# vrettasm/VGPA

Hardware: AMD Instinct MI355X
Metric: fwd+bwd sweeps/sec (free-energy+grad eval), Lorenz96 D=40 N=1000 (higher is better)
Workload: dtype f64; 1 GPU; Lorenz96 D=40, RK4, Np=1001 (BASELINE configs[2]); batch_per_gpu=512, kernels=mfma

## Files before the change

vgpa_amd/csrc/ode_sym_impl.h:

```cpp
#pragma once
#include <type_traits>
#include <utility>
#include "ode_mfma_impl.h"

namespace vgpa {
namespace sym {

using mfma::cdiv;
using mfma::cmax;
using mfma::cmin;
using mfma::d2_t;
using mfma::ldg;
using mfma::ldu;
using mfma::n_stages;
using mfma::settle;
using mfma::stage_op;
using mfma::stg;
using mfma::OP_M;
using mfma::OP_R;
using mfma::OP_X;

constexpr int kMaxNB = 16;

struct Run { int c, j0, j1; };
// ... 21 lines not shown
        if (j == v || (cov & pair_bit(v, j))) continue;
        if (a < 0) a = j;
        else if (b < 0) b = j;
      }
      if (b < 0) break;
      cov |= pair_bit(v, a) | pair_bit(v, b);
      if (n == want) res = Run{v, a, b};
      n++;
    }
  }
  for (int v = 0; v < nsb; v++)
    for (int j = v + 1; j < nsb; j++) {
      if (cov & pair_bit(v, j)) continue;
      cov |= pair_bit(v, j);
      if (n == want) res = Run{v, j, -1};
      n++;
    }
  if (count) *count = n;
  return res;
}

__host__ __device__ constexpr int sym_run_count(int nsb) {
  int n = 0;
  (void)sym_run(nsb, -2, &n);
  return n;
}

constexpr int kCoverPat[4][2] = {{0, 2}, {0, 3}, {1, 2}, {1, 3}};
constexpr int kCoverMaps[4][4][4] = {
    {{1, 8, 6, 1}, {2, 6, 7, 3}, {6, 5, 5, 4}, {9, 2, 5, 2}},
    {{9, 9, 8, 0}, {8, 1, 1, 2}, {8, 1, 1, 2}, {4, 5, 0, 5}},
    {{6, 9, 3, 6}, {4, 0, 5, 9}, {4, 0, 5, 9}, {0, 7, 4, 3}},
    {{8, 1, 7, 8}, {6, 7, 2, 3}, {6, 7, 2, 3}, {7, 3, 4, 0}}};
constexpr int kCoverUsed[4] = {0xB, 0xF, 0xF, 0xF};
constexpr bool kCoverAlias[4] = {false, true, true, true};
constexpr int kCoverLoopSlot = 2;
__host__ __device__ constexpr bool cover_slot_used(int w, int s) { return (kCoverUsed[w] >> s) & 1; }
__host__ __device__ constexpr bool cover_owner(int w, int s, int q) {
  const int I = kCoverMaps[w][kCoverPat[s][0]][q], J = kCoverMaps[w][kCoverPat[s][1]][q];
  const int lo = I < J ? I : J, hi = I < J ? J : I;
  for (int w2 = 0; w2 <= w; w2++)
    for (int s2 = 0; s2 < 4; s2++)
      for (int q2 = 0; q2 < 4; q2++) {
        if (!cover_slot_used(w2, s2)) continue;
        if (w2 == w && (s2 > s || (s2 == s && q2 >= q))) return true;
        const int I2 = kCoverMaps[w2][kCoverPat[s2][0]][q2], J2 = kCoverMaps[w2][kCoverPat[s2][1]][q2];
        if ((I2 < J2 ? I2 : J2) == lo && (I2 < J2 ? J2 : I2) == hi) return false;
      }
  return true;
}
struct CoverOwnerTab { unsigned char m[4][4]; };
__host__ __device__ constexpr CoverOwnerTab cover_owner_tab() {
  CoverOwnerTab t{};
  for (int w = 0; w < 4; w++)
    for (int s = 0; s < 4; s++) {
      unsigned char bits = 0;
      for (int q = 0; q < 4; q++)
        if (cover_slot_used(w, s) && cover_owner(w, s, q)) bits = (unsigned char)(bits | (1u << q));
      t.m[w][s] = bits;
    }
  return t;
}
__device__ constexpr CoverOwnerTab kCoverOwner = cover_owner_tab();
__host__ __device__ constexpr int cover_pairs_owned() {
  int n = 0;
  for (int w = 0; w < 4; w++)
    for (int s = 0; s < 4; s++)
      for (int q = 0; q < 4; q++) n += (cover_slot_used(w, s) && cover_owner(w, s, q)) ? 1 : 0;
  return n;
}
static_assert(cover_pairs_owned() == 55, "the fragment cover must own every block pair of the 10 x 10 upper triangle exactly once");
__host__ __device__ constexpr bool cover_diagonals_in_loop_units() {
  for (int w = 0; w < 4; w++)
    for (int s = 0; s < 4; s++)
      for (int q = 0; q < 4; q++) {
        if (!cover_slot_used(w, s)) continue;
        const bool diag = kCoverMaps[w][kCoverPat[s][0]][q] == kCoverMaps[w][kCoverPat[s][1]][q];
        const bool loop = kCoverAlias[w] && s == kCoverLoopSlot;
        if (diag != loop) return false;
      }
  return !cover_slot_used(0, kCoverLoopSlot);
}
static_assert(cover_diagonals_in_loop_units(), "single-chain loop units: every diagonal block in slot 2 of a triangle wave, slot 2 of the rectangle wave unused");

template <int NB_>
struct SGeo {
  static constexpr int NB = NB_;
  static constexpr int NW = 4, NT = 64 * NW;
  static constexpr int P = 4 * NB;
  static constexpr int NSB = (NB + 1) / 2;
  static constexpr int KKE = 2 * NSB;
  static constexpr int PP = 4 * KKE;
  static constexpr int RP = 2 * KKE;
  static constexpr int NKP = NSB;
  static constexpr int LD = 32 * cdiv(2 * PP - 16, 32) + 16;
  static constexpr int XS = RP * LD;
  static constexpr int NRUNS = sym_run_count(NSB);
  static constexpr int NR = cdiv(NRUNS, 4);
  static constexpr int MAXS = 2 * NR;
  static constexpr int XV = PP + 4;
  static constexpr int NPARTF = cmin(NT / PP, RP);
  static constexpr int RPP = cdiv(RP, NPARTF);
  static constexpr int NPF = cmin(NPARTF, cdiv(RP, RPP));
  static constexpr int NCB = PP / 4;
  static constexpr int NPARTB = cmin(NT / RP, NCB);
  static constexpr int CBP = cdiv(NCB, NPARTB);
  static constexpr int NPART = cmax(NPF, NPARTB);
  static constexpr int PV = NPART * PP;
  static constexpr int NIT = cdiv((P / 2) * P, NT);
  static constexpr int NTILE = cdiv(P / 2, 8) * cdiv(P, 8);
  static constexpr int NITF = cdiv(NTILE, NW);
  static constexpr size_t LDS_DOUBLES = (size_t)4 * XS + NW * XV + 2 * PV + 2 * NT;
  static_assert(NPARTF >= 1 && NPARTB >= 1, "dimension too large for the workgroup");
};

template <int NB>
__host__ __device__ constexpr int elem_off(int k, int c) {
  return (k >> 1) * SGeo<NB>::LD + 2 * (c ^ ((k >> 1) & 3)) + (k & 1);
}
template <int NB>
__host__ __device__ constexpr int unit_off(int p, int c) {
  return p * SGeo<NB>::LD + 2 * (c ^ (p & 3));
}

template <int NB>
struct ItemTab {
  static constexpr int NIT = SGeo<NB>::NIT;
  int lo[NIT];
  unsigned g0[NIT];
  unsigned g1[NIT];
  bool two[NIT];
  bool st0[NIT], st1[NIT];
};
template <int NB>
__device__ __forceinline__ void build_items(int D, int tid, ItemTab<NB>& T, bool packed_lower = false) {
  using g = SGeo<NB>;
#pragma unroll
  for (int q = 0; q < g::NIT; q++) {
    const int e = tid + g::NT * q;
    const int p = e / g::P, c = e - p * g::P;
    const bool ok = 2 * p < D && c < D;
    T.lo[q] = ok ? unit_off<NB>(p, c) : -1;
    T.g0[q] = ok ? 8u * (unsigned)(2 * p * D + c) : 0u;
    T.two[q] = ok && 2 * p + 1 < D;
    T.g1[q] = T.two[q] ? T.g0[q] + 8u * (unsigned)D : T.g0[q];
    T.st0[q] = ok; T.st1[q] = T.two[q];
    if (packed_lower) {
      const int r0 = 2 * p, r1 = 2 * p + 1;
      T.st0[q] = ok && c <= r0;
      T.st1[q] = T.two[q] && c <= r1;
      T.g0[q] = T.st0[q] ? 8u * (unsigned)(r0 * (r0 + 1) / 2 + c) : 0u;
      T.g1[q] = T.st1[q] ? 8u * (unsigned)(r1 * (r1 + 1) / 2 + c) : 0u;
    }
  }
}

template <int NB>
struct TileTab {
  static constexpr int NIT = SGeo<NB>::NITF;
  int lo[NIT];
  unsigned g0[NIT], g1[NIT];
  bool two[NIT];
};
template <int NB>
__device__ __forceinline__ void build_tiles(int D, int wave, int lane, TileTab<NB>& T) {
  using g = SGeo<NB>;
// ... 263 lines not shown
      for (int u = 0; u < 6; u++) wr1(eo_o[u], __builtin_fma(m2dt, gacc[u], -(uu[u / 3] * mm[u % 3])));
    } else {
#pragma unroll
      for (int u = 0; u < 7; u++) wr1(eo_o[u], __builtin_fma(m2dt, gacc[u], -(uu[u < 3 ? u : 2] * mm[u < 3 ? 0 : u - 2])));
    }
  };
  auto out = [&](int tg) {
    double* gA = gbase + (size_t)tg * DD;
    double v[NOUT];
#pragma unroll
    for (int q = 0; q < NOUT; q++) v[q] = rd1(ol[q]);
#pragma unroll
    for (int q = 0; q < NOUT; q++) stgo(gA, oo[q], v[q]);
  };
  using I0 = std::integral_constant<int, 0>; using I1 = std::integral_constant<int, 1>; using I2 = std::integral_constant<int, 2>;
  using I4 = std::integral_constant<int, 4>; using I5 = std::integral_constant<int, 5>;

  constexpr int kPrio = 3;
  auto step = [&](int k, auto set_, auto hp_, auto hp2_) {
    constexpr int SET = decltype(set_)::value;
    constexpr bool HP = decltype(hp_)::value, HP2 = decltype(hp2_)::value;
    using CUR = std::integral_constant<int, SET>; using PRV = std::integral_constant<int, SET ^ 1>;
    opaque_tables();
    if (HP) settle_loads();
    if (HP2) out(tidx(k - 2));
    __builtin_amdgcn_sched_barrier(0);
    build(CUR{});
    __builtin_amdgcn_sched_barrier(0);
    if (HP) prod(PRV{}, I0{}, I1{});
    lds_barrier();
    band_u(CUR{}, tidx(k));
    prefetch(tidx(k + 1));
    __builtin_amdgcn_sched_barrier(0);
    if (HP) prod(PRV{}, I1{}, I2{});
    lds_barrier();
    if (HP) prod(PRV{}, I2{}, I4{});
    lds_barrier();
    if (HP) { prod(PRV{}, I4{}, I5{}); __builtin_amdgcn_sched_barrier(0); epilogue(PRV{}); }
    lds_barrier();
  };
  auto drain = [&](auto set_) {
    constexpr int SET = decltype(set_)::value;
    using CUR = std::integral_constant<int, SET>; using PRV = std::integral_constant<int, SET ^ 1>;
    if (n_steps > 0) settle_loads();
    if (n_steps > 1) out(tidx(n_steps - 2));
    build(CUR{});
    if (n_steps > 0) prod(PRV{}, I0{}, I5{});
    lds_barrier();
    if (n_steps > 0) epilogue(PRV{});
    band_u(CUR{}, tidx(n_steps));
    lds_barrier();
    if (n_steps > 0) out(tidx(n_steps - 1));
    prod(CUR{}, I0{}, I5{});
    lds_barrier();
    epilogue(CUR{});
    lds_barrier();
    out(tidx(n_steps));
  };

  __builtin_amdgcn_s_setprio(kPrio);
  __syncthreads();
  prefetch(tidx(0));
  settle_loads();
  __syncthreads();
  using F = std::false_type; using T = std::true_type;
  int k = 0;
  if (n_steps > 0) { step(0, I0{}, F{}, F{}); k = 1; }
  if (n_steps > 1) { step(1, I1{}, T{}, F{}); k = 2; }
  for (; k + 1 < n_steps; k += 2) { step(k, I0{}, T{}, T{}); step(k + 1, I1{}, T{}, T{}); }
  if (k < n_steps) step(k, I0{}, T{}, T{});
  if (n_steps & 1) drain(I1{});
  else drain(I0{});
}

template <int METHOD, bool FWD, int NB, bool DENSEJ, int GR, int WPE, bool QOUT = false, bool HLP = false, bool GF = false, bool H2 = false, bool PJ = false>
__global__ void __attribute__((amdgpu_flat_work_group_size(256 * ((GF || H2) ? 3 : (HLP ? 2 : 1)), 256 * ((GF || H2) ? 3 : (HLP ? 2 : 1))), amdgpu_waves_per_eu(WPE, WPE))) k_ode_sym(OdeArgs a) {
#pragma clang fp contract(fast)
  extern __shared__ __attribute__((aligned(16))) double smem[];
  using g = SGeo<NB>;
  constexpr int NT = g::NT;
  constexpr int NS = n_stages<METHOD>(), NR = g::NR, MAXS = g::MAXS, LD = g::LD, NKP = g::NKP;
  constexpr bool COVER = (GR == 0);
  static_assert(!COVER || (g::NSB == 5 && g::MAXS == 4), "the fragment cover is built for 33 <= D <= 40");
  static_assert(!HLP || COVER, "helper waves: fragment-cover kernels");
  static_assert(!GF || (HLP && QOUT && !FWD && !DENSEJ && METHOD == VGPA_ODE_RK4), "fused gradient assembly: backward RK4 helper-wave kernels with Q'' on");
  static_assert(!H2 || (HLP && !GF), "two helper roles: helper-wave kernels without the gradient waves");
  static_assert(!PJ || (!FWD && !DENSEJ), "per-problem constant matrix jump: backward kernels with sparse jumps");
  constexpr int NITS = FWD ? g::NITF : g::NIT;
  constexpr int JSEC = NS > 1 ? 1 : 0;
  constexpr int LSTG = (NS == 4 && HLP) ? 3 : JSEC;
  constexpr double sixth = 1.0 / 6.0;
  const int role = HLP ? (int)threadIdx.x / NT : 0;
  const bool helper = role >= 1;
  const int tid = (int)threadIdx.x - role * NT, lane = tid & 63, wave = tid >> 6;
  const int wq = wave & 3;
  const int prob = (int)blockIdx.x;
  const int D = a.D, Np = a.Np, DD = a.D * a.D, n_steps = a.Np - 1;
  const double dt = a.dt, h = 0.5 * a.dt;
  const double q_scale = a.q_scale_v ? lds_const(a.q_scale_v, prob) : a.q_scale;
  double* const Xb0 = smem;
  double* const Xb1 = Xb0 + g::XS;
  double* const Rb = Xb1 + g::XS;
  double* const Mb = Rb + g::XS;
  double* const xvw = Mb + g::XS + wave * g::XV;
  double* const pvb = Mb + g::XS + g::NW * g::XV;
  double* const trash = pvb + 2 * g::PV + 2 * tid;
  using gl = GradLds<NB>;
  constexpr int GLDS = GF ? gl::DOUBLES : 0;
  if constexpr (GF) {
    if (role == 2) { grad_waves<NB>(a, smem, (int)threadIdx.x - 2 * NT); return; }
  }
  double* const gLam = smem + g::LDS_DOUBLES + gl::LAM;
  for (int i = tid; i < (int)g::LDS_DOUBLES + GLDS; i += NT) smem[i] = 0.0;
  static_assert(!QOUT || (!FWD && (METHOD == VGPA_ODE_RK2 || METHOD == VGPA_ODE_RK4)), "Q'' is stored by the backward mid-point kernels");
  auto tidx =[&](int i) { return FWD ? i : Np - 1 - i; };
  auto tclamp = [&](int i) { return tidx(i <= n_steps ? i : n_steps); };

  const int r4 = lane >> 4, bq = (lane >> 2) & 3, c4 = lane & 3, bi = bq >> 1, bj = bq & 1;
  int colI[NR], colJ[MAXS], offD[MAXS], offM[MAXS];
  int colm[4] = {0, 0, 0, 0};
  unsigned gofs[MAXS];
  bool own[MAXS], wd[MAXS], wm[MAXS];
  const int cov_used = COVER ? kCoverUsed[wq] : 0;
  const bool loop_diag = r4 == c4;
  const int loop_src = 16 * c4 + 4 * bq + r4;
  if constexpr (COVER) {
#pragma unroll
    for (int m = 0; m < 4; m++) colm[m] = 2 * ((4 * kCoverMaps[wq][m][bq] + c4) ^ r4);
#pragma unroll
    for (int s = 0; s < MAXS; s++) {
      const int Ib = kCoverMaps[wq][kCoverPat[s][0]][bq], Jb = kCoverMaps[wq][kCoverPat[s][1]][bq];
      const int row = 4 * Ib + r4, col = 4 * Jb + c4;
      const bool first = (kCoverOwner.m[wq][s] >> bq) & 1u;
      const bool act = ((cov_used >> s) & 1) && first && (Ib != Jb || row <= col);
      offD[s] = elem_off<NB>(row, col);
      offM[s] = elem_off<NB>(col, row);
      wd[s] = act;
      wm[s] = act && row != col;
      own[s] = act && row < D && col < D;
      gofs[s] = own[s] ? 8u * (unsigned)(row <= col ? row * D + col : col * D + row) : 0u;
      if (!FWD && a.ds_packed) gofs[s] = own[s] ? 8u * (unsigned)(row <= col ? tri_off(col) + row : tri_off(row) + col) : 0u;
      colJ[s] = 0;
    }
#pragma unroll
    for (int rl = 0; rl < NR; rl++) colI[rl] = 0;
  } else {
#pragma unroll
  for (int rl = 0; rl < NR; rl++) {
    const Run run = sym_run(g::NSB, wave + 4 * rl, nullptr);
    const bool rv = run.c >= 0;
    const int c = rv ? run.c : 0;
    const int Ib = 2 * c + bi;
    colI[rl] = 2 * ((4 * Ib + c4) ^ r4);
#pragma unroll
    for (int t = 0; t < 2; t++) {
      const int s = 2 * rl + t;
      const int jr = t ? run.j1 : run.j0;
      const bool valid = rv && jr >= 0;
      const int j = valid ? jr : 0;
      const int Jb = 2 * j + bj;
      const int row = 4 * Ib + r4, col = 4 * Jb + c4;
      colJ[s] = 2 * ((4 * Jb + c4) ^ r4);
      offD[s] = elem_off<NB>(row, col);
      offM[s] = elem_off<NB>(col, row);
      const bool act = valid && (c != j || row <= col);
      wd[s] = act;
      wm[s] = act && row != col;
      own[s] = act && row < D && col < D;
      gofs[s] = own[s] ? 8u * (unsigned)(row <= col ? row * D + col : col * D + row) : 0u;
      if (!FWD && a.ds_packed) gofs[s] = own[s] ? 8u * (unsigned)(row <= col ? tri_off(col) + row : tri_off(row) + col) : 0u;
    }
  }
  }
  const bool spk = FWD && a.s_packed;
  const int MS = spk ? D * (D + 1) / 2 : DD;
  ItemTab<NB> IT;
  build_items<NB>(D, tid, IT, spk);
  TileTab<NB> TT;
  if (FWD) build_tiles<NB>(D, wave, lane, TT);

  const double* A = a.A + (size_t)prob * a.strideA;
  d2_t an[NITS];
  auto load_a = [&](const double* At) {
#pragma unroll
    for (int q = 0; q < NITS; q++) {
      an[q][0] = ldgo(At, FWD ? TT.g0[q] : IT.g0[q]);
      an[q][1] = ldgo(At, FWD ? TT.g1[q] : IT.g1[q]);
    }
  };
  auto unit_ptr = [&](double* buf, int q) -> d2_t* {
    const int lo = FWD ? TT.lo[q] : IT.lo[q];
    return reinterpret_cast<d2_t*>(lo >= 0 ? buf + lo : trash);
  };
  auto mask_a = [&]() {
#pragma unroll
    for (int q = 0; q < NITS; q++)
      if (!(FWD ? TT.two[q] : IT.two[q])) an[q][1] = 0.0;
  };
  auto store_a = [&](double* buf, const d2_t (&v)[NITS]) {
#pragma unroll
    for (int q = 0; q < NITS; q++) *unit_ptr(buf, q) = v[q];
  };
  const int GS = (!FWD && a.ds_packed) ? D * (D + 1) / 2 : DD;
  const double* G = FWD ? a.Sigma + (size_t)prob * a.Sigma_stride : a.dEs + (size_t)prob * Np * GS;
  double* const mout = (FWD ? a.S : a.psi) + (size_t)prob * Np * (spk ? D * (D + 1) / 2 : DD);
  double xk[MAXS], acc[MAXS], fc[MAXS], fn[MAXS], fnn[MAXS];
#pragma unroll
  for (int s = 0; s < MAXS; s++) {
// ... 4 lines not shown
    acc[s] = 0.0;
  }

  const bool vl = lane < D;
  unsigned lane8 = vl ? 8u * (unsigned)lane : 0u;
  double* const xv_mine = vl ? xvw + lane : trash;
  const double* cin = FWD ? a.b + (size_t)prob * a.strideB : a.dEm + (size_t)prob * Np * D;
  double* const vout = (FWD ? a.m : a.lam) + (size_t)prob * Np * D;
  auto vec = [&](int t) { return (size_t)t * D; };
  const bool sparse_j = !FWD && !DENSEJ && a.obs_idx && a.jm_sparse;
  const int32_t* const obs_idx = a.obs_idx + (size_t)prob * a.obs_idx_stride;
  auto jump_vector = [&](int t, int n_obs) -> double {
    if (!FWD && DENSEJ) return ldg(a.jm_dense + ((size_t)prob * Np + t) * D, lane8);
    if (sparse_j && __builtin_amdgcn_readfirstlane(n_obs) >= 0) return ldg(a.jm_sparse + ((size_t)prob * a.n_obs + n_obs) * D, lane8);
    return 0.0;
  };
  double vk = FWD ? ldg(a.m0 + (size_t)prob * a.m0_stride, lane8) : 0.0, v1 = 0.0;
  double c0 = ldg(cin + vec(tidx(0)), lane8), c1 = ldg(cin + vec(tclamp(1)), lane8), c2 = 0.0;
  int n_obs_cur = sparse_j ? ldu(obs_idx, tclamp(1)) : -1, n_obs_next = sparse_j ? ldu(obs_idx, tclamp(2)) : -1, n_obs_nn = -1;
  double jm = n_steps >= 1 ? jump_vector(tidx(1), n_obs_cur) : 0.0, jm_next = 0.0;

  __syncthreads();
#pragma unroll
  for (int s = 0; s < MAXS; s++) {
    if (FWD) {
      *(wd[s] ? Xb0 + offD[s] : trash) = xk[s];
      *(wm[s] ? Xb0 + offM[s] : trash) = xk[s];
    }
  }
  *xv_mine = vk;
  load_a(A + (size_t)tidx(0) * DD);
  mask_a();
  store_a(Rb, an);
  load_a(A + (size_t)tclamp(1) * DD);
#pragma unroll
  for (int s = 0; s < MAXS; s++) { settle(fc[s]); settle(fn[s]); settle(xk[s]); }
  settle(c0); settle(c1); settle(vk); settle(jm);
#pragma unroll
  for (int q = 0; q < NITS; q++) settle(an[q]);
  mask_a();
  auto mask_f = [&](int s, double v) -> double {
    if (COVER && s == kCoverLoopSlot) v *= loop_diag ? 0.5 : 1.0;
    return own[s] ? -v : 0.0;
  };
#pragma unroll
  for (int s = 0; s < MAXS; s++) { fc[s] = mask_f(s, fc[s]); if (!FWD) fn[s] = mask_f(s, fn[s]); }
  __syncthreads();

  auto store_vector = [&](int t) {
    if (wave == 0 && vl) stgo(vout + vec(t), lane8, vk);
  };
  auto store_items = [&](const d2_t (&v)[g::NIT], int t, bool with_vector = true) {
    double* so = mout + (size_t)t * MS;
#pragma unroll
    for (int q = 0; q < g::NIT; q++) {
      if (IT.st0[q]) stgo(so, IT.g0[q], v[q][0]);
      if (IT.st1[q]) stgo(so, IT.g1[q], v[q][1]);
    }
    if (with_vector) store_vector(t);
  };
  auto load_items = [&](const double* Xc, d2_t (&v)[g::NIT]) {
#pragma unroll
    for (int q = 0; q < g::NIT; q++) v[q] = *reinterpret_cast<const d2_t*>(IT.lo[q] >= 0 ? Xc + IT.lo[q] : trash);
  };

  auto prefetch = [&](int step, auto helper_role) {
    constexpr int HK = decltype(helper_role)::value;
    constexpr bool ch_a = !HLP || HK == 1 || HK == 3, ch_v = !HLP || HK == 1 || HK == 2, units = !HLP || HK == 0;
    if (LSTG == JSEC) {
      if (ch_a) load_a(A + (size_t)tclamp(step + 2) * DD);
      if (ch_v) c2 = ldgo(cin + vec(tclamp(step + 2)), lane8);
    }
    if (!FWD) {
      if (units) {
#pragma unroll
        for (int s = 0; s < MAXS; s++) fnn[s] = ldgo(G + (size_t)tclamp(step + 2) * GS, gofs[s]);
      }
      if (ch_v) jm_next = step + 2 <= n_steps ? jump_vector(tidx(step + 2), n_obs_next) : 0.0;
      n_obs_nn = (sparse_j && step + 3 <= n_steps) ? ldu(obs_idx, tidx(step + 3)) : -1;
    }
  };

  constexpr int NAV = FWD ? g::RPP : 4 * g::CBP;
  constexpr int NPS = FWD ? g::NPF : g::NPARTB;
  d2_t tb_av[NAV], tb_xqf[FWD ? g::RPP : 1];
  double tb_xqb[FWD ? 1 : 4 * g::CBP];
  d2_t tc_mid[NITS], tc_items[g::NIT];
  double ta_ps[NPS];
  const int pdiv = FWD ? g::PP : g::RP;
  const int tb_part0 = tid / pdiv, tb_idx = tid - tb_part0 * pdiv;
  const bool tb_act = tb_part0 < (FWD ? g::NPF : g::NPARTB);
  const int tb_part = tb_act ? tb_part0 : 0;
  constexpr bool TB_FULL = FWD ? (g::NPF * g::RPP == g::RP) : (g::NPARTB * g::CBP == g::NCB);
  auto tailB_read = [&](const double* Aop) {
    if (FWD) {
#pragma unroll
      for (int r = 0; r < g::RPP; r++) {
        const int rp0 = tb_part * g::RPP + r;
        const int rp = rp0 < g::RP ? rp0 : 0;
        tb_av[r] = *reinterpret_cast<const d2_t*>(Aop + unit_off<NB>(rp, tb_idx));
        tb_xqf[r] = *reinterpret_cast<const d2_t*>(xvw + 2 * rp);
      }
    } else {
#pragma unroll
      for (int q = 0; q < g::CBP; q++) {
        const int cbq = tb_part + q * g::NPARTB;
        int cb = (cbq < g::NCB ? cbq : 0) + (tb_idx >> 2);
        if (cb >= g::NCB) cb -= g::NCB;
#pragma unroll
        for (int kk = 0; kk < 4; kk++) {
          tb_av[4 * q + kk] = *reinterpret_cast<const d2_t*>(Aop + tb_idx * LD + 2 * (4 * cb + (kk ^ (tb_idx & 3))));
          tb_xqb[4 * q + kk] = xvw[4 * cb + kk];
        }
      }
    }
  };
  auto tailB_finish = [&](double* pv) {
    double s0 = 0.0, s1 = 0.0;
    if (FWD) {
#pragma unroll
      for (int r = 0; r < g::RPP; r++) {
        const bool in = TB_FULL || tb_part * g::RPP + r < g::RP;
        s0 = __builtin_fma(tb_av[r][0], in ? tb_xqf[r][0] : 0.0, s0);
        s0 = __builtin_fma(tb_av[r][1], in ? tb_xqf[r][1] : 0.0, s0);
      }
      *(tb_act ? pv + tb_part * g::PP + tb_idx : trash) = s0;
    } else {
#pragma unroll
      for (int q = 0; q < g::CBP; q++) {
        const bool in = TB_FULL || tb_part + q * g::NPARTB < g::NCB;
#pragma unroll
        for (int kk = 0; kk < 4; kk++) {
          const double xv = in ? tb_xqb[4 * q + kk] : 0.0;
          s0 = __builtin_fma(tb_av[4 * q + kk][0], xv, s0);
          s1 = __builtin_fma(tb_av[4 * q + kk][1], xv, s1);
        }
      }
      d2_t o; o[0] = s0; o[1] = s1;
      *reinterpret_cast<d2_t*>(tb_act ? pv + tb_part * g::PP + 2 * tb_idx : trash) = o;
    }
  };
  constexpr bool MIDP = (METHOD == VGPA_ODE_RK2 || METHOD == VGPA_ODE_RK4);
  auto tailC_read = [&](int j, const double* Xc) {
    if (j == 0) {
      if (MIDP) {
#pragma unroll
        for (int q = 0; q < NITS; q++) tc_mid[q] = *unit_ptr(Rb, q);
      }
      if constexpr (!GF) load_items(Xc, tc_items);
    }
  };
  auto to_q = [&](d2_t (&items)[g::NIT], const d2_t (&a0)[NITS]) {
    if constexpr (QOUT) {
      const double qs = q_scale;
#pragma unroll
      for (int q = 0; q < g::NIT; q++) {
        items[q][0] = __builtin_fma(qs, a0[q][0], -2.0 * items[q][0]);
        items[q][1] = __builtin_fma(qs, a0[q][1], -2.0 * items[q][1]);
      }
    }
  };
  using K1 = std::integral_constant<int, 1>; using K2 = std::integral_constant<int, 2>; using K3 = std::integral_constant<int, 3>;
  auto tailC_finish = [&](int j, int step, auto kind_) {
    constexpr int KIND = decltype(kind_)::value;
    if (j == 0) {
      double* dst = (METHOD == VGPA_ODE_EULER && (step & 1)) ? Rb : Mb;
      if constexpr (QOUT && !GF) to_q(tc_items, tc_mid);
      if (MIDP) {
#pragma unroll
        for (int q = 0; q < NITS; q++) { tc_mid[q][0] = 0.5 * (tc_mid[q][0] + an[q][0]); tc_mid[q][1] = 0.5 * (tc_mid[q][1] + an[q][1]); }
        store_a(dst, tc_mid);
      } else {
        store_a(dst, an);
      }
      if constexpr (GF) {
        if (wave == 0 && vl) { stgo(vout + vec(tidx(step)), lane8, vk); gLam[lane] = vk; }
      } else if (!(KIND == 3 && NS > 1)) store_items(tc_items, tidx(step), KIND == 1);
    }
    if (KIND == 3 && NS > 1 && j == (NS > 2 ? 2 : 1)) store_items(tc_items, tidx(step), false);
    if (j == JSEC && NS > 1) store_a(Rb, an);
    if (j == JSEC) prefetch(step, kind_);
    if (LSTG != JSEC && j == LSTG) {
      load_a(A + (size_t)tclamp(step + 2) * DD);
      if (KIND == 1) c2 = ldgo(cin + vec(tclamp(step + 2)), lane8);
    }
  };
  auto vec_chores = [&](int j, int step) {
    if (j == 0) store_vector(tidx(step));
    if (j == JSEC) prefetch(step, K2{});
    if (LSTG != JSEC && j == LSTG) c2 = ldgo(cin + vec(tclamp(step + 2)), lane8);
  };

  auto vecA_read = [&](const double* pv) {
    const double* pl = pv + (vl ? lane : 0);
#pragma unroll
    for (int q = 0; q < NPS; q++) ta_ps[q] = pl[q * g::PP];
  };
  auto vecA_finish = [&](int j) {
    double vs = ta_ps[0];
#pragma unroll
    for (int q = 1; q < NPS; q++) vs += ta_ps[q];
    const double cmid = 0.5 * (c0 + c1);
    double vn;
    if (METHOD == VGPA_ODE_EULER) { vk = vk + (c0 - vs) * dt + jm; vn = vk; }
    else if (METHOD == VGPA_ODE_HEUN) {
      if (j == 0) { v1 = c0 - vs; vn = vk + v1 * dt; }
      else { vk = vk + h * (v1 + (c1 - vs)) + jm; vn = vk; }
    } else if (METHOD == VGPA_ODE_RK2) {
      if (j == 0) vn = vk + h * (c0 - vs);
      else { vk = vk + dt * (cmid - vs) + jm; vn = vk; }
    } else {
      if (j == 0) { v1 = c0 - vs; vn = vk + h * v1; }
      else if (j == 1) { const double f = cmid - vs; v1 = v1 + 2.0 * f; vn = vk + h * f; }
      else if (j == 2) { const double f = cmid - vs; v1 = v1 + 2.0 * f; vn = vk + dt * f; }
      else { vk = vk + (dt * (v1 + (c1 - vs))) * sixth + jm; vn = vk; }
    }
    *xv_mine = vn;
  };

  auto element = [&](int s, int j, double z, double js) -> double {
    const double f = -z;
    double xn;
    if (METHOD == VGPA_ODE_EULER) { xk[s] = xk[s] + f * dt + js; xn = xk[s]; }
    else if (METHOD == VGPA_ODE_HEUN) {
      if (j == 0) { acc[s] = f; xn = xk[s] + f * dt; }
      else { xk[s] = xk[s] + h * (acc[s] + f) + js; xn = xk[s]; }
    } else if (METHOD == VGPA_ODE_RK2) {
      if (j == 0) xn = xk[s] + h * f;
      else { xk[s] = xk[s] + dt * f + js; xn = xk[s]; }
    } else {
      if (j == 0) { acc[s] = f; xn = xk[s] + h * f; }
      else if (j == 1) { acc[s] = acc[s] + 2.0 * f; xn = xk[s] + h * f; }
      else if (j == 2) { acc[s] = acc[s] + 2.0 * f; xn = xk[s] + dt * f; }
      else { xk[s] = xk[s] + (dt * (acc[s] + f)) * sixth + js; xn = xk[s]; }
    }
    return xn;
  };

  constexpr int GRR = COVER ? 1 : GR;
  constexpr int NG = COVER ? 1 : cdiv(NR, GRR), NSL = COVER ? 4 : 2 * GRR, NSTEP = NG * NKP;
  static_assert(COVER || NR % GRR == 0, "a group of runs must be complete (the clamped tail group is not parity-clean)");
  d2_t fa1[2][GRR], fa2[2][GRR], fb1[2][COVER ? 1 : NSL], fb2[2][COVER ? 1 : NSL];
  constexpr bool HALF = COVER && !HLP && !FWD;
  d2_t fAa, fXa, fAb[2][COVER ? 2 : 1], fXb[2][COVER ? 2 : 1];
  d2_t fAa1[2], fXa1[2];
  d2_t fA[2][(COVER && !HALF) ? 4 : 1], fX[2][(COVER && !HALF) ? 4 : 1];
  auto frag_all = [&](int buf, int kp, const double* pa, const double* px) {
#pragma unroll
    for (int m = 0; m < 4; m++) {
      fA[buf][m] = *reinterpret_cast<const d2_t*>(pa + kp * 4 * LD + colm[m]);
      fX[buf][m] = *reinterpret_cast<const d2_t*>(px + kp * 4 * LD + colm[m]);
    }
  };
  auto frag_a0 = [&](int kp, const double* pa, const double* px) {
    fAa = *reinterpret_cast<const d2_t*>(pa + kp * 4 * LD + colm[0]);
    fXa = *reinterpret_cast<const d2_t*>(px + kp * 4 * LD + colm[0]);
  };
  auto frag_a1 = [&](int buf, int kp, const double* pa, const double* px) {
    fAa1[buf] = *reinterpret_cast<const d2_t*>(pa + kp * 4 * LD + colm[1]);
    fXa1[buf] = *reinterpret_cast<const d2_t*>(px + kp * 4 * LD + colm[1]);
  };
  auto frag_b = [&](int buf, int kp, const double* pa, const double* px) {
#pragma unroll
    for (int m = 0; m < 2; m++) {
      fAb[buf][m] = *reinterpret_cast<const d2_t*>(pa + kp * 4 * LD + colm[2 + m]);
      fXb[buf][m] = *reinterpret_cast<const d2_t*>(px + kp * 4 * LD + colm[2 + m]);
    }
  };
  auto frag_load = [&](int buf, int t, const double* pa, const double* px) {
    if constexpr (COVER) {
      const int kp = t % NKP;
      if constexpr (HALF) {
        frag_a0(kp, pa, px);
        frag_b(buf, kp, pa, px);
        frag_a1(buf, kp, pa, px);
      } else {
        frag_all(buf, kp, pa, px);
      }
    } else {
      const int g0 = (t / NKP) * GRR, kp = t % NKP;
#pragma unroll
      for (int r = 0; r < GRR; r++) {
        const int rl = g0 + r < NR ? g0 + r : NR - 1;
        fa1[buf][r] = *reinterpret_cast<const d2_t*>(pa + kp * 4 * LD + colI[rl]);
        fa2[buf][r] = *reinterpret_cast<const d2_t*>(px + kp * 4 * LD + colI[rl]);
      }
#pragma unroll
      for (int u = 0; u < NSL; u++) {
        const int sl = 2 * g0 + u < MAXS ? 2 * g0 + u : MAXS - 1;
        fb1[buf][u] = *reinterpret_cast<const d2_t*>(px + kp * 4 * LD + colJ[sl]);
        fb2[buf][u] = *reinterpret_cast<const d2_t*>(pa + kp * 4 * LD + colJ[sl]);
      }
    }
  };
  auto product_begin = [&](const double* Aop, const double* Xc) {
    frag_load(0, 0, Aop + r4 * LD, Xc + r4 * LD);
  };

  auto product_stage = [&](int j, int step, const double* Aop, const double* Xc, double* Xn, auto&& chore) {
    const double* pa = Aop + r4 * LD;
    const double* px = Xc + r4 * LD;
    const bool last = (j == NS - 1);
    const bool jump_now = !FWD && last && !DENSEJ && __builtin_amdgcn_readfirstlane(n_obs_cur) >= 0;
    double jsd[MAXS];
    if (!FWD && last && DENSEJ) {
#pragma unroll
      for (int s = 0; s < MAXS; s++) jsd[s] = ldgo(a.js_dense + ((size_t)prob * Np + tidx(step + 1)) * DD, gofs[s]);
    }
    if (!FWD && last && !DENSEJ) {
#pragma unroll
      for (int s = 0; s < MAXS; s++) jsd[s] = 0.0;
      if (jump_now && a.js_const) {
#pragma unroll
        for (int s = 0; s < MAXS; s++) jsd[s] = ldgo(PJ ? a.js_const + (size_t)prob * a.js_const_stride : a.js_const, gofs[s]);
      }
    }
    double w[NSL];
    chore(-1);
#pragma unroll
    for (int t = 0; t < NSTEP; t++) {
      const int gi = t / NKP, kp = t % NKP, g0 = gi * GRR, cur = t & 1;
      if (!COVER && t + 1 < NSTEP) frag_load(cur ^ 1, t + 1, pa, px);
      if (kp == 0) {
#pragma unroll
        for (int u = 0; u < NSL; u++) {
          const int s = 2 * g0 + u;
          double f = 0.0;
          if (s < MAXS) {
            if (FWD || METHOD == VGPA_ODE_EULER) f = fc[s];
            else if (METHOD == VGPA_ODE_HEUN) f = j == 0 ? fc[s] : fn[s];
            else if (METHOD == VGPA_ODE_RK2) f = j == 0 ? fc[s] : 0.5 * (fn[s] + fc[s]);
            else f = j == 0 ? fc[s] : (j == 3 ? fn[s] : 0.5 * (fn[s] + fc[s]));
          }
          w[u] = f;
        }
      }
      if constexpr (COVER) {
        if constexpr (!HALF) {
          __builtin_amdgcn_sched_barrier(0);
          if (t + 1 < NSTEP) frag_all(cur ^ 1, (t + 1) % NKP, pa, px);
#pragma unroll
          for (int hh = 0; hh < 2; hh++) {
#pragma unroll
            for (int u = 0; u < 4; u++) w[u] = __builtin_amdgcn_mfma_f64_4x4x4f64(fA[cur][u >> 1][hh], fX[cur][2 + (u & 1)][hh], w[u], 0, 0, 0);
#pragma unroll
            for (int u = 0; u < 4; u++)
              if (u != kCoverLoopSlot) w[u] = __builtin_amdgcn_mfma_f64_4x4x4f64(fX[cur][u >> 1][hh], fA[cur][2 + (u & 1)][hh], w[u], 0, 0, 0);
          }
          if (t + 1 < NSTEP) {
#pragma unroll
            for (int i = 0; i < 6; i++) {
              __builtin_amdgcn_sched_group_barrier(0x008, 2, 0);
              __builtin_amdgcn_sched_group_barrier(0x100, 1, 0);
            }
#pragma unroll
            for (int i = 0; i < 2; i++) {
              __builtin_amdgcn_sched_group_barrier(0x008, 1, 0);
              __builtin_amdgcn_sched_group_barrier(0x100, 1, 0);
            }
          }
          __builtin_amdgcn_sched_barrier(0);
        } else {
          __builtin_amdgcn_sched_barrier(0);
          if (t + 1 < NSTEP) { frag_b(cur ^ 1, (t + 1) % NKP, pa, px); frag_a1(cur ^ 1, (t + 1) % NKP, pa, px); }
#pragma unroll
          for (int hh = 0; hh < 2; hh++) {
#pragma unroll
            for (int m = 0; m < 2; m++) w[m] = __builtin_amdgcn_mfma_f64_4x4x4f64(fAa[hh], fXb[cur][m][hh], w[m], 0, 0, 0);
#pragma unroll
            for (int m = 0; m < 2; m++) w[m] = __builtin_amdgcn_mfma_f64_4x4x4f64(fXa[hh], fAb[cur][m][hh], w[m], 0, 0, 0);
          }
          if (t + 1 < NSTEP) {
#pragma unroll
            for (int i = 0; i < 6; i++) {
              __builtin_amdgcn_sched_group_barrier(0x008, 1, 0);
              __builtin_amdgcn_sched_group_barrier(0x100, 1, 0);
            }
          }
          __builtin_amdgcn_sched_barrier(0);
          if (t + 1 < NSTEP) frag_a0((t + 1) % NKP, pa, px);
#pragma unroll
          for (int hh = 0; hh < 2; hh++) {
            w[3] = __builtin_amdgcn_mfma_f64_4x4x4f64(fAa1[cur][hh], fXb[cur][1][hh], w[3], 0, 0, 0);
            w[2] = __builtin_amdgcn_mfma_f64_4x4x4f64(fAa1[cur][hh], fXb[cur][0][hh], w[2], 0, 0, 0);
            w[3] = __builtin_amdgcn_mfma_f64_4x4x4f64(fXa1[cur][hh], fAb[cur][1][hh], w[3], 0, 0, 0);
          }
          if (t + 1 < NSTEP) {
            __builtin_amdgcn_sched_group_barrier(0x008, 2, 0);
            __builtin_amdgcn_sched_group_barrier(0x100, 1, 0);
            __builtin_amdgcn_sched_group_barrier(0x008, 2, 0);
            __builtin_amdgcn_sched_group_barrier(0x100, 1, 0);
          }
          __builtin_amdgcn_sched_barrier(0);
        }
      } else {
#pragma unroll
      for (int hh = 0; hh < 2; hh++) {
#pragma unroll
        for (int u = 0; u < NSL; u++) w[u] = __builtin_amdgcn_mfma_f64_4x4x4f64(fa1[cur][u >> 1][hh], fb1[cur][u][hh], w[u], 0, 0, 0);
#pragma unroll
        for (int u = 0; u < NSL; u++) w[u] = __builtin_amdgcn_mfma_f64_4x4x4f64(fa2[cur][u >> 1][hh], fb2[cur][u][hh], w[u], 0, 0, 0);
      }
      }
      chore(t);
      if (kp == NKP - 1) {
        if constexpr (COVER) {
          w[kCoverLoopSlot] += __shfl(w[kCoverLoopSlot], loop_src, 64);
        }
#pragma unroll
        for (int u = 0; u < NSL; u++) {
          const int s = 2 * g0 + u;
          if (s < MAXS) {
            double js = 0.0;
            if (!FWD && last) js = own[s] ? jsd[s] : 0.0;
            const double xn = element(s, j, w[u], js);
            *(wd[s] ? Xn + offD[s] : trash) = xn;
            *(wm[s] ? Xn + offM[s] : trash) = xn;
          }
        }
      }
    }
  };

  auto xcur = [&](int k, int j) -> double* { return (((NS & 1) ? (k & 1) : (j & 1)) ? Xb1 : Xb0); };
  auto aop = [&](int k, int j, bool matrix) -> const double* {
    const int op = stage_op<METHOD, FWD>(j, matrix, k);
    return op == OP_X ? xcur(k, j) : (op == OP_M ? Mb : Rb);
  };
  if (role == 0) product_begin(aop(0, 0, true), xcur(0, 0));
  constexpr int LAST = NSTEP - 1;
  constexpr bool SPLIT = COVER;
  constexpr bool SPA = SPLIT, SPC = SPLIT && FWD;
  constexpr int TBU = NSTEP >= 5 ? NSTEP / 4 + 1 : (NSTEP > 1 ? 1 : 0), TCU = NSTEP >= 5 ? NSTEP / 2 + 1 : LAST;
  constexpr int SA_F = 0, SA_R = SPA ? -1 : SA_F;
  constexpr int SB_F = SPLIT ? cmin(1, LAST) : TBU, SB_R = SB_F;
  constexpr int SC_F = SPLIT ? cmin(2, LAST) : TCU, SC_R = SPC ? cmin(1, LAST) : SC_F;
  auto time_loop = [&](auto helper_role) {
  constexpr int HK = HLP ? decltype(helper_role)::value : 0;
  constexpr bool HR = HK != 0;
  for (int k = 0; k < n_steps; k++) {
    if (k > 0) {
      if (!HLP || HK == 1 || HK == 3) {
#pragma unroll
        for (int q = 0; q < NITS; q++) settle(an[q]);
        mask_a();
      }
      if (!FWD) {
        if (!HR) {
#pragma unroll
          for (int s = 0; s < MAXS; s++) { fc[s] = fn[s]; fn[s] = mask_f(s, fnn[s]); }
        }
        n_obs_cur = n_obs_next; n_obs_next = n_obs_nn;
      }
    }
#pragma unroll
    for (int j = 0; j < NS; j++) {
      const double* Xc = xcur(k, j);
      double* Xn = (Xc == Xb0) ? Xb1 : Xb0;
      double* pv = pvb + (Xc == Xb0 ? 0 : g::PV);
      double* pv_prev = pvb + (Xc == Xb0 ? g::PV : 0);
      const double* Aopv = aop(k, j, false);
      if constexpr (HR) {
        if (HK != 3 && (j > 0 || k > 0)) vecA_read(pv_prev);
        if (HK != 2) tailC_read(j, Xc);
        if (HK != 3) {
          if (j > 0) vecA_finish(j - 1);
          else if (k > 0) {
            vecA_finish(NS - 1);
            c0 = c1; c1 = c2;
            if (!FWD) jm = jm_next;
          }
          tailB_read(Aopv);
          tailB_finish(pv);
        }
        if (HK == 1) tailC_finish(j, k, K1{});
        if (HK == 2) vec_chores(j, k);
        if (HK == 3) tailC_finish(j, k, K3{});
      } else
      product_stage(j, k, aop(k, j, true), Xc, Xn, [&](int t) {
        if (HLP) {
          if (t == SC_F && j == JSEC) prefetch(k, std::false_type{});
          return;
        }
        if (SPLIT) __builtin_amdgcn_sched_barrier(0);
        if (t == SA_R && (j > 0 || k > 0)) vecA_read(pv_prev);
        if (t == SA_F) {
          if (j > 0) vecA_finish(j - 1);
          else if (k > 0) {
            vecA_finish(NS - 1);
            c0 = c1; c1 = c2;
            if (!FWD) jm = jm_next;
          }
        }
        if (t == SB_R) tailB_read(Aopv);
        if (t == SB_F) tailB_finish(pv);
        if (t == SC_R) tailC_read(j, Xc);
        if (t == SC_F) tailC_finish(j, k, K1{});
        if (SPLIT) __builtin_amdgcn_sched_barrier(0);
      });
      __builtin_amdgcn_s_setprio(1);
      lds_barrier();
      const int kn = j + 1 < NS ? k : k + 1, jn = j + 1 < NS ? j + 1 : 0;
      if (!HR) product_begin(aop(kn, jn, true), Xn);
      __builtin_amdgcn_s_setprio(0);
    }
  }
  };
  if (H2 && role == 1) time_loop(K2{});
  else if (H2 && role == 2) time_loop(K3{});
  else if (HLP && helper) time_loop(K1{});
  else time_loop(std::integral_constant<int, 0>{});
  if constexpr (GF) {
    if (role == 0) { lds_barrier(); lds_barrier(); lds_barrier(); lds_barrier(); return; }
  }
  if (HLP && !helper) return;
  if (!(H2 && role == 2) && n_steps > 0) {
    vecA_read(pvb + (xcur(n_steps, 0) == Xb0 ? g::PV : 0));
    vecA_finish(NS - 1);
  }
  if (H2 && role == 1) { store_vector(tidx(n_steps)); return; }
  if constexpr (GF) {
    if (wave == 0 && vl) { stgo(vout + vec(tidx(n_steps)), lane8, vk); gLam[lane] = vk; }
    lds_barrier(); lds_barrier(); lds_barrier(); lds_barrier();
  } else {
    d2_t items[g::NIT];
    load_items(xcur(n_steps, 0), items);
    if constexpr (QOUT) {
      d2_t a0[NITS];
#pragma unroll
      for (int q = 0; q < NITS; q++) a0[q] = *unit_ptr(Rb, q);
      to_q(items, a0);
    }
    store_items(items, tidx(n_steps), !H2);
  }
}


struct SymVariant {
  bool dense;
  bool q_out;
  bool own_jump;
  bool grad;
  int helper_roles;
};

template <int METHOD, bool FWD, int NB>
constexpr bool sym_variant_exists(SymVariant v) {
  constexpr bool cover = SGeo<NB>::NSB == 5;
  constexpr bool midpoint = METHOD == VGPA_ODE_RK2 || METHOD == VGPA_ODE_RK4;
  if (FWD && (v.dense || v.q_out || v.own_jump || v.grad)) return false;
  if (v.dense && (v.q_out || v.own_jump || v.grad)) return false;
  if (v.q_out && !(midpoint && cover)) return false;
  if (v.grad && !(METHOD == VGPA_ODE_RK4 && v.q_out && v.helper_roles == 1)) return false;
  return v.helper_roles == 0 || (cover && (v.helper_roles == 1 || v.helper_roles == 2));
}

template <int METHOD, int NB>
constexpr bool sym_variant_rules_hold() {
  constexpr bool cover = SGeo<NB>::NSB == 5, midpoint = METHOD == VGPA_ODE_RK2 || METHOD == VGPA_ODE_RK4;
  for (int bits = 0; bits < 16; bits++)
    for (int roles = 0; roles <= 2; roles++) {
      const SymVariant v{(bits & 1) != 0, (bits & 2) != 0, (bits & 4) != 0, (bits & 8) != 0, roles};
      if (sym_variant_exists<METHOD, true, NB>(v) && (v.dense || v.q_out || v.own_jump || v.grad)) return false;
      if (!sym_variant_exists<METHOD, false, NB>(v)) continue;
      if (v.grad && !v.q_out) return false;
      if (v.q_out && !(midpoint && cover)) return false;
      if (roles > 0 && !cover) return false;
    }
  for (int D = 4 * NB - 3; D <= 4 * NB; D++) {
    if (stores_q(METHOD, D) != sym_variant_exists<METHOD, false, NB>(SymVariant{false, true, false, false, 0})) return false;
    if (fuses_grad(METHOD, D) != sym_variant_exists<METHOD, false, NB>(SymVariant{false, true, false, true, 1})) return false;
  }
  return true;
}
template <int... I>
constexpr bool sym_variant_rules_hold_everywhere(std::integer_sequence<int, I...>) {
  return (... && sym_variant_rules_hold<I / kMaxNB, I % kMaxNB + 1>());
}
static_assert(sym_variant_rules_hold_everywhere(std::make_integer_sequence<int, 4 * kMaxNB>{}),
              "k_ode_sym variants: forward kernels take no backward option, grad => q_out, q_out => RK2 / RK4 on the cover, helper roles => "
              "the cover, and stores_q / fuses_grad say the same");

struct SymLaunchShape { int threads, gr, wpe; size_t lds; };
template <int NB>
constexpr SymLaunchShape sym_launch_shape(SymVariant v) {
  const int sets = 1 + v.helper_roles + (v.grad ? 1 : 0);
  const size_t lds = (SGeo<NB>::LDS_DOUBLES + (v.grad ? GradLds<NB>::DOUBLES : 0)) * sizeof(double);
  return {256 * sets, SGeo<NB>::NSB == 5 ? 0 : 1, sets > 1 ? sets : (2 * lds <= 160 * 1024 ? 2 : 1), lds};
}

template <int METHOD, bool FWD, int NB, bool DENSE, bool QOUT, bool PJ, bool GRAD, int ROLES>
hipError_t launch_variant(const OdeArgs& a, hipStream_t st) {
  constexpr SymVariant V{DENSE, QOUT, PJ, GRAD, ROLES};
  if constexpr (sym_variant_exists<METHOD, FWD, NB>(V)) {
// ... 56 lines not shown
```

Before: 21990 sweeps/s.

## Compute forward A·v with MFMA inside the product waves' fragment cover

In forward cover kernels, the matrix-vector product A v is now computed by the product waves with extra 4x4x4 f64 MFMAs on the fragments they already load. Publishing lanes write each row block of the result once into the partial-vector buffer, replacing the scalar tailB read/finish path. On wave 0 the skipped diagonal loop-slot MFMAs are dropped, and the schedule-group barriers are retuned for the new MFMA and read mix. This removes separate LDS reads and scalar FMA work for the vector chain, but adds MFMA and register pressure to the product waves' critical path.

```diff
diff --git a/vgpa_amd/csrc/ode_sym_impl.h b/vgpa_amd/csrc/ode_sym_impl.h
--- a/vgpa_amd/csrc/ode_sym_impl.h
+++ b/vgpa_amd/csrc/ode_sym_impl.h
@@ -127,6 +127,19 @@
   return !cover_slot_used(0, kCoverLoopSlot);
 }
 static_assert(cover_diagonals_in_loop_units(), "single-chain loop units: every diagonal block in slot 2 of a triangle wave, slot 2 of the rectangle wave unused");
+
+constexpr int kCoverVecMap = 1;
+constexpr int kCoverVecBlocks[4] = {0xF, 0x3, 0xF, 0x0};
+__host__ __device__ constexpr bool cover_vec_rows_once() {
+  int cnt[10] = {};
+  for (int w = 0; w < 4; w++)
+    for (int q = 0; q < 4; q++)
+      if ((kCoverVecBlocks[w] >> q) & 1) cnt[kCoverMaps[w][kCoverVecMap][q]]++;
+  for (int i = 0; i < 10; i++)
+    if (cnt[i] != 1) return false;
+  return true;
+}
+static_assert(cover_vec_rows_once(), "the vector chain's publishing blocks must hold every row block of A v exactly once");
 
 template <int NB_>
 struct SGeo {
@@ -556,6 +569,7 @@
   constexpr int NS = n_stages<METHOD>(), NR = g::NR, MAXS = g::MAXS, LD = g::LD, NKP = g::NKP;
   constexpr bool COVER = (GR == 0);
   static_assert(!COVER || (g::NSB == 5 && g::MAXS == 4), "the fragment cover is built for 33 <= D <= 40");
+  constexpr bool VMC = COVER && FWD;
   static_assert(!HLP || COVER, "helper waves: fragment-cover kernels");
   static_assert(!GF || (HLP && QOUT && !FWD && !DENSEJ && METHOD == VGPA_ODE_RK4), "fused gradient assembly: backward RK4 helper-wave kernels with Q'' on");
   static_assert(!H2 || (HLP && !GF), "two helper roles: helper-wave kernels without the gradient waves");
@@ -598,6 +612,8 @@
   const int cov_used = COVER ? kCoverUsed[wq] : 0;
   const bool loop_diag = r4 == c4;
   const int loop_src = 16 * c4 + 4 * bq + r4;
+  const int vrow = COVER ? 4 * kCoverMaps[wq][kCoverVecMap][bq] + r4 : 0;
+  const bool vpub = VMC && c4 == 0 && ((kCoverVecBlocks[wq] >> bq) & 1);
   if constexpr (COVER) {
 #pragma unroll
     for (int m = 0; m < 4; m++) colm[m] = 2 * ((4 * kCoverMaps[wq][m][bq] + c4) ^ r4);
@@ -768,7 +784,7 @@
   };
 
   constexpr int NAV = FWD ? g::RPP : 4 * g::CBP;
-  constexpr int NPS = FWD ? g::NPF : g::NPARTB;
+  constexpr int NPS = VMC ? 1 : (FWD ? g::NPF : g::NPARTB);
   d2_t tb_av[NAV], tb_xqf[FWD ? g::RPP : 1];
   double tb_xqb[FWD ? 1 : 4 * g::CBP];
   d2_t tc_mid[NITS], tc_items[g::NIT];
@@ -882,7 +898,7 @@
 #pragma unroll
     for (int q = 0; q < NPS; q++) ta_ps[q] = pl[q * g::PP];
   };
-  auto vecA_finish = [&](int j) {
+  auto vecA_finish = [&](int j, bool publish = true) {
     double vs = ta_ps[0];
 #pragma unroll
     for (int q = 1; q < NPS; q++) vs += ta_ps[q];
@@ -901,7 +917,7 @@
       else if (j == 2) { const double f = cmid - vs; v1 = v1 + 2.0 * f; vn = vk + dt * f; }
       else { vk = vk + (dt * (v1 + (c1 - vs))) * sixth + jm; vn = vk; }
     }
-    *xv_mine = vn;
+    if (publish) *xv_mine = vn;
   };
 
   auto element = [&](int s, int j, double z, double js) -> double {
@@ -931,6 +947,15 @@
   d2_t fAa, fXa, fAb[2][COVER ? 2 : 1], fXb[2][COVER ? 2 : 1];
   d2_t fAa1[2], fXa1[2];
   d2_t fA[2][(COVER && !HALF) ? 4 : 1], fX[2][(COVER && !HALF) ? 4 : 1];
+  d2_t fV[VMC ? NKP : 1], fA0, fAs[VMC ? NKP : 1];
+  double wv = 0.0;
+  auto vec_frags = [&](bool sep, const double* Aopv) {
+#pragma unroll
+    for (int kp = 0; kp < (VMC ? NKP : 0); kp++) {
+      fV[kp] = *reinterpret_cast<const d2_t*>(xvw + 8 * kp + 2 * r4);
+      if (sep) fAs[kp] = *reinterpret_cast<const d2_t*>(Aopv + (4 * kp + r4) * LD + colm[kCoverVecMap]);
+    }
+  };
   auto frag_all = [&](int buf, int kp, const double* pa, const double* px) {
 #pragma unroll
     for (int m = 0; m < 4; m++) {
@@ -983,7 +1008,10 @@
     frag_load(0, 0, Aop + r4 * LD, Xc + r4 * LD);
   };
 
-  auto product_stage = [&](int j, int step, const double* Aop, const double* Xc, double* Xn, auto&& chore) {
+  auto product_stage = [&](int j, int step, const double* Aop, const double* Xc, double* Xn, double* pv, bool sep, auto vc_, auto&& chore) {
+    constexpr int VC = decltype(vc_)::value;
+    constexpr bool VCH = VMC && VC != 2;
+    constexpr bool NO2 = VMC && VC == 0;
     const double* pa = Aop + r4 * LD;
     const double* px = Xc + r4 * LD;
     const bool last = (j == NS - 1);
@@ -1025,15 +1053,30 @@
         if constexpr (!HALF) {
           __builtin_amdgcn_sched_barrier(0);
           if (t + 1 < NSTEP) frag_all(cur ^ 1, (t + 1) % NKP, pa, px);
+          if (VCH && t == 0) wv = 0.0;
+          if (VCH && !sep && t == 1) fA0 = *reinterpret_cast<const d2_t*>(pa + colm[kCoverVecMap]);
+          if (VCH && (t == 2 || t == 3)) wv = __builtin_amdgcn_mfma_f64_4x4x4f64(sep ? fAs[0][t - 2] : fA0[t - 2], fV[0][t - 2], wv, 0, 0, 0);
 #pragma unroll
           for (int hh = 0; hh < 2; hh++) {
 #pragma unroll
-            for (int u = 0; u < 4; u++) w[u] = __builtin_amdgcn_mfma_f64_4x4x4f64(fA[cur][u >> 1][hh], fX[cur][2 + (u & 1)][hh], w[u], 0, 0, 0);
+            for (int u = 0; u < 4; u++)
+              if (!(NO2 && u == kCoverLoopSlot)) w[u] = __builtin_amdgcn_mfma_f64_4x4x4f64(fA[cur][u >> 1][hh], fX[cur][2 + (u & 1)][hh], w[u], 0, 0, 0);
 #pragma unroll
             for (int u = 0; u < 4; u++)
               if (u != kCoverLoopSlot) w[u] = __builtin_amdgcn_mfma_f64_4x4x4f64(fX[cur][u >> 1][hh], fA[cur][2 + (u & 1)][hh], w[u], 0, 0, 0);
+            if (VCH && t >= 1) wv = __builtin_amdgcn_mfma_f64_4x4x4f64(sep ? fAs[VMC ? kp : 0][hh] : fA[cur][kCoverVecMap][hh], fV[VMC ? kp : 0][hh], wv, 0, 0, 0);
           }
-          if (t + 1 < NSTEP) {
+          if (VMC && t + 1 < NSTEP) {
+            const int nm = 14 - (NO2 ? 2 : 0) + (VCH ? (t >= 1 ? 2 : 0) + ((t == 2 || t == 3) ? 1 : 0) : 0), nr = 8 + ((VCH && !sep && t == 1) ? 1 : 0);
+            const int two = nm - nr < nr ? nm - nr : nr;
+#pragma unroll
+            for (int i = 0; i < 9; i++)
+              if (i < nr) {
+                if (i < two) __builtin_amdgcn_sched_group_barrier(0x008, 2, 0);
+                else __builtin_amdgcn_sched_group_barrier(0x008, 1, 0);
+                __builtin_amdgcn_sched_group_barrier(0x100, 1, 0);
+              }
+          } else if (t + 1 < NSTEP) {
 #pragma unroll
             for (int i = 0; i < 6; i++) {
               __builtin_amdgcn_sched_group_barrier(0x008, 2, 0);
@@ -1090,13 +1133,14 @@
       }
       chore(t);
       if (kp == NKP - 1) {
-        if constexpr (COVER) {
+        if constexpr (COVER && !NO2) {
           w[kCoverLoopSlot] += __shfl(w[kCoverLoopSlot], loop_src, 64);
         }
+        if constexpr (VCH) *(vpub ? pv + vrow : trash) = wv;
 #pragma unroll
         for (int u = 0; u < NSL; u++) {
           const int s = 2 * g0 + u;
-          if (s < MAXS) {
+          if (s < MAXS && !(NO2 && s == kCoverLoopSlot)) {
             double js = 0.0;
             if (!FWD && last) js = own[s] ? jsd[s] : 0.0;
             const double xn = element(s, j, w[u], js);
@@ -1121,7 +1165,8 @@
   constexpr int SA_F = 0, SA_R = SPA ? -1 : SA_F;
   constexpr int SB_F = SPLIT ? cmin(1, LAST) : TBU, SB_R = SB_F;
   constexpr int SC_F = SPLIT ? cmin(2, LAST) : TCU, SC_R = SPC ? cmin(1, LAST) : SC_F;
-  auto time_loop = [&](auto helper_role) {
+  auto time_loop = [&](auto helper_role, auto vc_) {
+  constexpr bool VCH = VMC && decltype(vc_)::value != 2;
   constexpr int HK = HLP ? decltype(helper_role)::value : 0;
   constexpr bool HR = HK != 0;
   for (int k = 0; k < n_steps; k++) {
@@ -1146,40 +1191,49 @@
       double* pv = pvb + (Xc == Xb0 ? 0 : g::PV);
       double* pv_prev = pvb + (Xc == Xb0 ? g::PV : 0);
       const double* Aopv = aop(k, j, false);
+      const bool sep = VMC && stage_op<METHOD, FWD>(j, true, k) != stage_op<METHOD, FWD>(j, false, k);
       if constexpr (HR) {
         if (HK != 3 && (j > 0 || k > 0)) vecA_read(pv_prev);
         if (HK != 2) tailC_read(j, Xc);
         if (HK != 3) {
+          if (j > 0) vecA_finish(j - 1, !VMC);
+          else if (k > 0) {
+            vecA_finish(NS - 1, !VMC);
+            c0 = c1; c1 = c2;
+            if (!FWD) jm = jm_next;
+          }
+          if (!VMC) {
+            tailB_read(Aopv);
+            tailB_finish(pv);
+          }
+        }
+        if (HK == 1) tailC_finish(j, k, K1{});
+        if (HK == 2) vec_chores(j, k);
+        if (HK == 3) tailC_finish(j, k, K3{});
+      } else
+      product_stage(j, k, aop(k, j, true), Xc, Xn, pv, sep, vc_, [&](int t) {
+        if (HLP && !VMC) {
+          if (t == SC_F && j == JSEC) prefetch(k, std::false_type{});
+          return;
+        }
+        if (SPLIT) __builtin_amdgcn_sched_barrier(0);
+        if ((!VMC || VCH) && t == SA_R && (j > 0 || k > 0)) vecA_read(pv_prev);
+        if ((!VMC || VCH) && t == SA_F) {
           if (j > 0) vecA_finish(j - 1);
           else if (k > 0) {
             vecA_finish(NS - 1);
             c0 = c1; c1 = c2;
             if (!FWD) jm = jm_next;
           }
-          tailB_read(Aopv);
-          tailB_finish(pv);
+          if (VMC) vec_frags(sep, Aopv);
         }
-        if (HK == 1) tailC_finish(j, k, K1{});
-        if (HK == 2) vec_chores(j, k);
-        if (HK == 3) tailC_finish(j, k, K3{});
-      } else
-      product_stage(j, k, aop(k, j, true), Xc, Xn, [&](int t) {
         if (HLP) {
-          if (t == SC_F && j == JSEC) prefetch(k, std::false_type{});
+          if (VCH && t == SC_F && j == JSEC) c2 = ldgo(cin + vec(tclamp(k + 2)), lane8);
+          if (SPLIT) __builtin_amdgcn_sched_barrier(0);
           return;
         }
-        if (SPLIT) __builtin_amdgcn_sched_barrier(0);
-        if (t == SA_R && (j > 0 || k > 0)) vecA_read(pv_prev);
-        if (t == SA_F) {
-          if (j > 0) vecA_finish(j - 1);
-          else if (k > 0) {
-            vecA_finish(NS - 1);
-            c0 = c1; c1 = c2;
-            if (!FWD) jm = jm_next;
-          }
-        }
-        if (t == SB_R) tailB_read(Aopv);
-        if (t == SB_F) tailB_finish(pv);
+        if (!VMC && t == SB_R) tailB_read(Aopv);
+        if (!VMC && t == SB_F) tailB_finish(pv);
         if (t == SC_R) tailC_read(j, Xc);
         if (t == SC_F) tailC_finish(j, k, K1{});
         if (SPLIT) __builtin_amdgcn_sched_barrier(0);
@@ -1192,10 +1246,15 @@
     }
   }
   };
-  if (H2 && role == 1) time_loop(K2{});
-  else if (H2 && role == 2) time_loop(K3{});
-  else if (HLP && helper) time_loop(K1{});
-  else time_loop(std::integral_constant<int, 0>{});
+  using K0 = std::integral_constant<int, 0>;
+  static_assert(!kCoverAlias[0] && kCoverVecBlocks[0] && kCoverVecBlocks[1] && kCoverVecBlocks[2] && !kCoverVecBlocks[3], "the product waves' vector roles below");
+  if (H2 && role == 1) time_loop(K2{}, K0{});
+  else if (H2 && role == 2) time_loop(K3{}, K0{});
+  else if (HLP && helper) time_loop(K1{}, K0{});
+  else if (!VMC) time_loop(K0{}, K0{});
+  else if (wq == 0) time_loop(K0{}, K0{});
+  else if (wq == 3) time_loop(K0{}, K2{});
+  else time_loop(K0{}, K1{});
   if constexpr (GF) {
     if (role == 0) { lds_barrier(); lds_barrier(); lds_barrier(); lds_barrier(); return; }
   }
```

After: 22260 sweeps/s, median of 6. 1.01x the previous value.
